# sanhue903/CUDA_Selection_Criteria

Measured on AMD Instinct MI355X. Metric: sketch pair-comparisons/sec (N genomes x m buckets), higher is better.
Workload: dtype u64; 1 GPU; cfg3: 10000 genomes, smh_a m=512, tau=0.8; mode smh_a; bands 64 x 8 rows; pair space sharded by query rows over 1 GPU(s), selected pairs all_gathered; n_genomes=10000, m=512, algo=sig, criterion=smh_a, selected_pairs=45000, stage1_survivors=45000, n_ranks_seen=1, stage2_grouping=label order

## Files before the change

cuda_selection_criteria_amd/csrc/abi_context.inc:

```

extern "C" {

const char* selhip_version(void) { return "selhip 0.1 (gfx950)"; }

int selhip_device_count(void) {
    int cnt = 0;
    if (hipGetDeviceCount(&cnt) != hipSuccess) return 0;
    return cnt;
}

const char* selhip_last_error(const selhip_ctx* ctx) {
    if (ctx) return ctx->err.c_str();
    return g_last_error.c_str();
}

int selhip_ctx_create(selhip_ctx** out, int device) {
    if (!out) return SELHIP_E_BADARG;
    *out = nullptr;
    int rc = check_device(nullptr);
    if (rc) return rc;
    int cnt = 0;
    (void)hipGetDeviceCount(&cnt);
    if (device < 0 || device >= cnt) { set_err(nullptr, "device %d out of range (0..%d)", device, cnt - 1); return SELHIP_E_BADARG; }
    HIPCHK(nullptr, hipSetDevice(device));
    hipDeviceProp_t prop;
    HIPCHK(nullptr, hipGetDeviceProperties(&prop, device));
    if (std::strncmp(prop.gcnArchName, "gfx950", 6) != 0) {
        set_err(nullptr, "device %d is %s; this library is built for gfx950 only", device, prop.gcnArchName);
        return SELHIP_E_NODEVICE;
    }
    selhip_ctx* c = new selhip_ctx();
    c->device = device;
    c->dev_cus = prop.multiProcessorCount;
    *out = c;
    return SELHIP_OK;
}

void selhip_ctx_destroy(selhip_ctx* c) {
    if (!c) return;
    (void)hipSetDevice(c->device);
    (void)hipStreamSynchronize(c->stream);
    drain_timers(c);
    c->own_hll.release(); c->own_aux.release(); c->own_cards.release();
    c->ecard.release(); c->hi.release(); c->pc.release(); c->seg_cnt.release(); c->surv.release();
    c->counts.release(); c->results.release(); c->self_pairs.release();
    c->aux_il.release(); c->cand.release(); c->sigQ.release(); c->sigT.release(); c->sigP.release(); c->sigG.release(); c->fin.release(); c->own_aux_hll.release();
    c->hj_keys_in.release(); c->hj_keys_out.release(); c->hj_vals_in.release(); c->hj_vals_out.release(); c->hj_tmp.release();
    c->csr_cnt.release(); c->csr_start.release(); c->grouped.release(); c->scan_tmp.release();
    c->hll_bs.release(); c->hll_bs_max.release(); c->hll_gmax.release(); c->small_bar.release();
    release_queries(c);
    if (c->h_pc) (void)hipHostFree(c->h_pc);
    if (c->st_stage1) {
        (void)hipStreamDestroy(c->st_stage1);
        (void)hipEventDestroy(c->ev_start); (void)hipEventDestroy(c->ev_end);
    }
    delete c;
}

int selhip_ctx_set_stream(selhip_ctx* c, void* hip_stream) {
    if (!c) return SELHIP_E_BADARG;
    if (c->stream != (hipStream_t)hip_stream && c->pc.p) {
        (void)hipStreamSynchronize(c->stream);
        c->pc_dirty = true;
    }
    c->stream = (hipStream_t)hip_stream;
    return SELHIP_OK;
}

int selhip_ctx_set_fp_mode(selhip_ctx* c, int fp_mode) {
    if (!c || (fp_mode != SELHIP_FP_FMA && fp_mode != SELHIP_FP_STRICT)) return SELHIP_E_BADARG;
    c->fp_mode = fp_mode;
    return SELHIP_OK;
}

int selhip_ctx_set_row_interleave(selhip_ctx* c, int block_rows, int n_parts, int part) {
    if (!c) return SELHIP_E_BADARG;
    if (n_parts <= 1) { c->il_parts = 1; c->il_part = 0; return SELHIP_OK; }
    if (block_rows < 32 || block_rows % 32 || part < 0 || part >= n_parts) {
        set_err(&c->err, "row interleave: block_rows must be a multiple of 32 (>= 32) and 0 <= part < n_parts");
        return SELHIP_E_BADARG;
    }
    c->il_block = block_rows; c->il_parts = n_parts; c->il_part = part;
// ... 60 lines not shown
        return SELHIP_OK;
    }
    if (!std::strcmp(name, "group_label")) {
        if (value < -1 || value > 1) { set_err(&c->err, "group_label must be -1 (automatic), 0 or 1"); return SELHIP_E_BADARG; }
        c->group_label = value;
        return SELHIP_OK;
    }
    if (!std::strcmp(name, "hist_run")) {
        if (value < 0 || value > 1024) { set_err(&c->err, "hist_run must be in [0, 1024] (0 = automatic)"); return SELHIP_E_BADARG; }
        c->hist_run = value;
        return SELHIP_OK;
    }
    if (!std::strcmp(name, "hist_pad")) {
        if (value < 0 || value > 48 * 1024) { set_err(&c->err, "hist_pad must be in [0, 49152]"); return SELHIP_E_BADARG; }
        c->hist_pad = value;
        return SELHIP_OK;
    }
    if (!std::strcmp(name, "query_join_tile")) {
        if (value != 16 && value != 32) { set_err(&c->err, "query_join_tile must be 16 or 32"); return SELHIP_E_BADARG; }
        c->query_join_tile = value;
        return SELHIP_OK;
    }
    if (!std::strcmp(name, "timed_kernel")) {
        if (value < 0 || value > 1) { set_err(&c->err, "timed_kernel must be 0 (stage-1 kernel) or 1 (stage 2a)"); return SELHIP_E_BADARG; }
        c->timed_kernel = value;
        return SELHIP_OK;
    }
    if (!std::strcmp(name, "hist_algo")) {
        if (value < -1 || value > 1) { set_err(&c->err, "hist_algo must be -1 (automatic), 0 (byte rows, LDS histogram) or 1 (bit planes)"); return SELHIP_E_BADARG; }
        c->hist_algo = value;
        if (value == 0) c->hll_khi = 0;
        return SELHIP_OK;
    }
    if (!std::strcmp(name, "hist_dense_degree")) {
        if (value < -1 || value > (1 << 20)) { set_err(&c->err, "hist_dense_degree must be in [-1, 2^20] (-1 = never)"); return SELHIP_E_BADARG; }
        c->hist_dense_degree = value;
        return SELHIP_OK;
    }
    if (!std::strcmp(name, "hist_bs_blocks")) {
        if (value < 8 || value > 65536 || value % 8) { set_err(&c->err, "hist_bs_blocks must be a multiple of 8 in [8, 65536]"); return SELHIP_E_BADARG; }
        c->hist_bs_blocks = value;
        return SELHIP_OK;
    }
    if (!std::strcmp(name, "hist_blocks")) {
        if (value < 8 || value > 65536 || value % 8) { set_err(&c->err, "hist_blocks must be a multiple of 8 in [8, 65536]"); return SELHIP_E_BADARG; }
        c->hist_blocks = value;
        return SELHIP_OK;
    }
    set_err(&c->err, "unknown parameter '%s'", name);
    return SELHIP_E_BADARG;
}

int selhip_ctx_get_param(const selhip_ctx* c, const char* name, int* value) {
    if (!c || !name || !value) return SELHIP_E_BADARG;
    if (!std::strcmp(name, "hll_khi"))          { *value = c->hll_khi; return SELHIP_OK; }
    if (!std::strcmp(name, "hist_bitplanes"))   { *value = use_bitslices(c) ? 1 : 0; return SELHIP_OK; }
    if (!std::strcmp(name, "label_order"))      { *value = label_order(c) ? 1 : 0; return SELHIP_OK; }
    if (!std::strcmp(name, "join_tile_rows"))   { *value = join_tile_rows(c); return SELHIP_OK; }
    if (!std::strcmp(name, "join_form_used"))   { *value = c->join_form_used; return SELHIP_OK; }
    if (!std::strcmp(name, "chunks"))           { *value = c->n_chunks_last; return SELHIP_OK; }
    if (!std::strcmp(name, "small_pass_used"))  { *value = c->small_used ? 1 : 0; return SELHIP_OK; }
    if (!std::strcmp(name, "query_db_sig_builds")) { *value = c->q.db_sig_builds; return SELHIP_OK; }
    return SELHIP_E_BADARG;
}

int selhip_ctx_set_candidate_begin(selhip_ctx* c, int64_t k_min) {
    if (!c) return SELHIP_E_BADARG;
    if (k_min < 0 || k_min > c->n) { set_err(&c->err, "candidate_begin %lld outside [0, n]", (long long)k_min); return SELHIP_E_BADARG; }
    c->cand_begin = k_min;
    return SELHIP_OK;
}

int selhip_ctx_set_stage2_grouping(selhip_ctx* c, int enable) {
    if (!c) return SELHIP_E_BADARG;
    c->group_stage2 = enable != 0;
    return SELHIP_OK;
}

int selhip_ctx_set_pipeline(selhip_ctx* c, int chunks) {
    if (!c || chunks < -1 || chunks > kMaxChunks) return SELHIP_E_BADARG;
    c->pipeline = chunks;
    return SELHIP_OK;
}

int selhip_ctx_set_criterion(selhip_ctx* c, int criterion) {
    if (!c || criterion < SELHIP_CRIT_SMH_A || criterion > SELHIP_CRIT_HLL_A_SMH_A) return SELHIP_E_BADARG;
    c->criterion = criterion;
    return SELHIP_OK;
}

int selhip_ctx_upload_aux_hll(selhip_ctx* c, const uint8_t* h_aux_hll, int p_aux) {
    if (!c || !h_aux_hll || p_aux < 4 || p_aux > kMaxAuxP) return SELHIP_E_BADARG;
    if (!c->d_hll && c->n) { set_err(&c->err, "upload the primary sketches first"); return SELHIP_E_STATE; }
    HIPCHK(&c->err, hipSetDevice(c->device));
    const size_t bytes = (size_t)c->n << p_aux;
    HIPCHK(&c->err, c->own_aux_hll.ensure(bytes ? bytes : 1));
    if (bytes) HIPCHK(&c->err, hipMemcpyAsync(c->own_aux_hll.p, h_aux_hll, bytes, hipMemcpyHostToDevice, c->stream));
    HIPCHK(&c->err, hipStreamSynchronize(c->stream));
    c->d_aux_hll = c->own_aux_hll.p; c->p_aux = p_aux;
    return SELHIP_OK;
}

int selhip_ctx_attach_aux_hll(selhip_ctx* c, const uint8_t* d_aux_hll, int p_aux) {
    if (!c || !d_aux_hll || p_aux < 4 || p_aux > kMaxAuxP) return SELHIP_E_BADARG;
    c->d_aux_hll = d_aux_hll; c->p_aux = p_aux;
    return SELHIP_OK;
}

static int validate_shape(selhip_ctx* c, int64_t n, int m, int p) {
    if (n < 0 || n > 0x7FFFFFF0ll) { set_err(&c->err, "n_genomes %lld out of range", (long long)n); return SELHIP_E_BADARG; }
    if (m <= 0) { set_err(&c->err, "m must be > 0"); return SELHIP_E_BADARG; }
    if (p < 4 || p > 20) { set_err(&c->err, "p_hll %d out of range [4,20]", p); return SELHIP_E_BADARG; }
    return SELHIP_OK;
}

static int after_sketches(selhip_ctx* c, const double* cards_src, bool cards_on_host) {
    c->hll_khi = 0;
    if (c->n == 0) return SELHIP_OK;
    if (c->p == 14 && c->hist_algo != 0) {
        HIPCHK(&c->err, c->hll_bs.ensure((size_t)c->n * kBsGenomeDwords));
        HIPCHK(&c->err, c->hll_bs_max.ensure(1));
        HIPCHK(&c->err, c->hll_gmax.ensure((size_t)c->n));
        const int rc = build_bitslices(&c->err, c->stream, c->d_hll, c->n, c->hll_bs.p, c->hll_gmax.p, c->hll_bs_max.p, &c->hll_khi);
        if (rc) return rc;
    }
    if (!cards_src) {
        HIPCHK(&c->err, c->own_cards.ensure((size_t)c->n));
        int rc = compute_cards(c, c->d_hll, c->n, c->p, c->own_cards.p);
        if (rc) return rc;
        c->d_cards = c->own_cards.p;
    } else if (cards_on_host) {
        for (int64_t i = 0; i < c->n; ++i) {
            double v = cards_src[i];
            if (!(v >= 0.0) || !(v < 9.2e18)) { set_err(&c->err, "cards[%lld] = %g is not a finite value in [0, 2^63)", (long long)i, v); return SELHIP_E_BADARG; }
            if (i && v < cards_src[i - 1]) { set_err(&c->err, "cards are not in ascending order at rank %lld", (long long)i); return SELHIP_E_BADARG; }
        }
        HIPCHK(&c->err, c->own_cards.ensure((size_t)c->n));
        HIPCHK(&c->err, hipMemcpyAsync(c->own_cards.p, cards_src, (size_t)c->n * sizeof(double), hipMemcpyHostToDevice, c->stream));
        c->d_cards = c->own_cards.p;
    } else {
        c->d_cards = cards_src;
    }
    HIPCHK(&c->err, hipStreamSynchronize(c->stream));
    return SELHIP_OK;
}

int selhip_ctx_upload(selhip_ctx* c, const uint8_t* h_hll, const uint64_t* h_aux, const double* h_cards,
                      int64_t n, int m, int p_hll) {
    if (!c) return SELHIP_E_BADARG;
    HIPCHK(&c->err, hipSetDevice(c->device));
    int rc = validate_shape(c, n, m, p_hll);
    if (rc) return rc;
    if (n > 0 && (!h_hll || !h_aux)) { set_err(&c->err, "null sketch pointer"); return SELHIP_E_BADARG; }
    c->n = n; c->m = m; c->p = p_hll; c->have_run = false; c->pending = false; c->cand_begin = 0; c->sig_key = 0; c->small_pass_failed = false;
    const size_t hb = (size_t)1 << p_hll;
    if (n > 0) {
// ... 242 lines not shown
```

cuda_selection_criteria_amd/csrc/host_context.hpp:

```cpp
#pragma once

namespace {

thread_local std::string g_last_error = "";

void set_err(std::string* dst, const char* fmt, ...) {
    char buf[512];
    va_list ap;
    va_start(ap, fmt);
    vsnprintf(buf, sizeof buf, fmt, ap);
    va_end(ap);
    if (dst) *dst = buf;
    g_last_error = buf;
}

#define HIPCHK(ctx_err, expr)                                                                  \
    do {                                                                                       \
        hipError_t e__ = (expr);                                                               \
        if (e__ != hipSuccess) {                                                               \
            set_err(ctx_err, "%s failed: %s (%s:%d)", #expr, hipGetErrorString(e__), __FILE__, __LINE__); \
            return SELHIP_E_HIP;                                                               \
        }                                                                                      \
    } while (0)

// ... 59 lines not shown
    DevBuf<selhip_int2_t> surv;
    DevBuf<uint32_t> counts;
    DevBuf<selhip_pair_t> results;
    DevBuf<selhip_int2_t> self_pairs;
    DevBuf<selhip_int2_t> cand;
    DevBuf<selhip_int2_t> fin;
    const uint8_t* d_aux_hll = nullptr;
    DevBuf<uint8_t> own_aux_hll;
    int p_aux = 0;
    int criterion = 0;
    DevBuf<u64> aux_il;
    DevBuf<uint32_t> sigQ, sigT, sigP, sigG;
    DevBuf<u64> hj_keys_in, hj_keys_out;
    DevBuf<int> hj_vals_in, hj_vals_out;
    DevBuf<char> hj_tmp;
    DevBuf<int> csr_cnt, csr_start;
    DevBuf<selhip_int2_t> grouped;
    DevBuf<char> scan_tmp;
    size_t scan_tmp_stride = 0;
    PassCounters* h_pc = nullptr;
    hipStream_t st_stage1 = nullptr;
    hipEvent_t ev_start = nullptr, ev_end = nullptr;
    int n_chunks_last = 1;
    int pipeline = -1;
    int64_t cand_begin = 0;
    int il_block = 128, il_parts = 1, il_part = 0;
    int hist_pad = 0;
    int hist_run = 0, hist_blocks = kHistSpanBlocks;
    DevBuf<uint32_t> hll_bs;
    DevBuf<u64> small_bar;
    DevBuf<uint8_t> hll_gmax;
    DevBuf<int> hll_bs_max;
    int hll_khi = 0;
    int hist_algo = -1;
    int hist_dense_degree = 32;
    int hist_bs_blocks = 2048;
    int group_label = -1;
    int verify_fb = 0;
    int join_wpb = 4;
    int join_db = 1;
    int join_tri = 0;
    int join_form = 2;
    int join_form_used = -1;
    int join_t = 0;
    int join_bits = 16;
    int join_q = 1;
    long long enum_pairs = kEnumPairs;
    int sig_tile_g = 16;
    int sig_cache = 0;
    long long sig_key = 0;
    int sig_tile = 1;
    int init_cap = 0;
    int join_qt = 0;
    bool group_stage2 = true;
    int small_pass = -1;
    bool small_used = false, small_pass_failed = false;
    int group_min_n = 2048;

    bool have_run = false, pending = false;
    int mode = 0, algo = 0, n_rows = 0, n_bands = 0;
    float tau_f = 0;
    int64_t row_begin = 0, row_end = 0;
    PassCounters last{};

    struct QuerySet {
        int64_t n = -1;
// ... 125 lines not shown
```

cuda_selection_criteria_amd/csrc/host_pass.hpp:

```cpp
#pragma once

namespace {

template <int NCH, int LOG2R>
hipError_t launch_stream(selhip_ctx* c, const StageIO& io, const RowMap& rm) {
    constexpr int Q = kQueryVgprBudget / NCH;
    const int n = (int)c->n;
    const long long n_tiles_ll = rm.n_tiles(Q);
    if (n_tiles_ll > 0x7FFFFFFFll) return hipErrorInvalidValue;
    const int n_tiles = (int)n_tiles_ll;
    const int chunk_base = ((rm.row_begin + 1) / kChunk) * kChunk;
    const int n_chunks = (n - chunk_base + kChunk - 1) / kChunk;
    if (n_tiles <= 0 || n_chunks <= 0) return hipSuccess;
    const long long blocks = (long long)n_tiles * n_chunks;
    if (blocks > 0x7FFFFFFFll) return hipErrorInvalidValue;
    hipLaunchKernelGGL((smh_stream_kernel<NCH, LOG2R>), dim3((unsigned)blocks), dim3(kBlock), 0, io.st,
                       reinterpret_cast<const u64x2*>(c->aux_il.p), n, c->hi.p, c->pcb,
                       rm, n_tiles, chunk_base, io.surv, io.cap, io.pc);
    return hipGetLastError();
}

template <int NCH, int LOG2R>
hipError_t launch_stream_r(selhip_ctx* c, const StageIO& io, int l, const RowMap& rm) {
    if (l == LOG2R) return launch_stream<NCH, LOG2R>(c, io, rm);
// ... 233 lines not shown
    size_t tmp_bytes = c->hj_tmp.cap;
    const unsigned end_bit = 32u + (unsigned)ilog2(n_bands) + 1u;
    e = rocprim::radix_sort_pairs(c->hj_tmp.p, tmp_bytes, c->hj_keys_in.p, c->hj_keys_out.p, c->hj_vals_in.p, c->hj_vals_out.p,
                                  (size_t)total, 0u, end_bit, io.st);
    if (e != hipSuccess) return e;
    hipLaunchKernelGGL(run_emit_kernel, dim3(grid_for((u64)total, kBlock, 8192)), dim3(kBlock), 0, io.st,
                       c->hj_keys_out.p, c->hj_vals_out.p, total, c->sigQ.p, n_bands, c->d_aux, c->m, n_rows, n_bands,
                       n, c->hi.p, c->pcb, rm, io.surv, io.cap, io.pc);
    return hipGetLastError();
}

template <int MODE>
hipError_t launch_select(bool fma, hipStream_t st, unsigned grid, const uint32_t* counts, const u64* n_dev, u64 n_host,
                         u64 cap, int p, double* est, const selhip_int2_t* pairs, const u64* ecard, double tau,
                         selhip_pair_t* results, u64 results_cap, PassCounters* pc,
                         selhip_result_t* rf32, int* out_count, u64 chunk_off = 0, u64 chunk_len = ~0ull) {
    const double rs = relerr_scaled_for(p);
    if (fma)
        hipLaunchKernelGGL((ertl_select_kernel<true, MODE>), dim3((grid + kWavesPerBlock - 1) / kWavesPerBlock), dim3(kBlock), 0, st, counts, n_dev, n_host, cap,
                           p, rs, est, pairs, ecard, tau, results, results_cap, pc, rf32, out_count, chunk_off, chunk_len);
    else
        hipLaunchKernelGGL((ertl_select_kernel<false, MODE>), dim3((grid + kWavesPerBlock - 1) / kWavesPerBlock), dim3(kBlock), 0, st, counts, n_dev, n_host, cap,
                           p, rs, est, pairs, ecard, tau, results, results_cap, pc, rf32, out_count, chunk_off, chunk_len);
    return hipGetLastError();
}

unsigned grid_for(u64 items, unsigned per_block, unsigned max_blocks) {
    u64 b = (items + per_block - 1) / per_block;
    if (b < 1) b = 1;
    if (b > max_blocks) b = max_blocks;
    return (unsigned)b;
}

hipError_t launch_hist_bs(int khi, unsigned blocks, hipStream_t st, const uint32_t* bs, const uint8_t* gmax, const selhip_int2_t* list, const u64* count,
                          u64 cap, uint32_t* counts, u64 off, u64 window, int run, u64 dense_pairs) {
#define SELHIP_BS_LAUNCH(NB) hipLaunchKernelGGL((hll_union_hist_bs_kernel<NB>), dim3(blocks), dim3(kBlock), 0, st, bs, gmax, list, count, cap, counts, off, window, run, dense_pairs)
    if (khi <= 16)      SELHIP_BS_LAUNCH(4);
    else if (khi <= 32) SELHIP_BS_LAUNCH(5);
    else                SELHIP_BS_LAUNCH(6);
#undef SELHIP_BS_LAUNCH
    return hipGetLastError();
}

int build_bitslices(std::string* err, hipStream_t st, const uint8_t* d_hll, int64_t n, uint32_t* d_bs, uint8_t* d_gmax, int* d_max, int* khi) {
    HIPCHK(err, hipMemsetAsync(d_max, 0, sizeof(int), st));
    hipLaunchKernelGGL(hll_bitslice_kernel, dim3(grid_for((u64)n, kWavesPerBlock, 8192)), dim3(kBlock), 0, st, d_hll, (long long)n, d_bs, d_gmax, d_max);
    HIPCHK(err, hipGetLastError());
    int mx = 0;
    HIPCHK(err, hipMemcpyAsync(&mx, d_max, sizeof(int), hipMemcpyDeviceToHost, st));
    HIPCHK(err, hipStreamSynchronize(st));
    *khi = mx + 1;
    return SELHIP_OK;
}

bool use_bitslices(const selhip_ctx* c) { return c->p == 14 && c->hll_khi > 0 && c->hist_algo != 0; }

int compute_cards(selhip_ctx* c, const uint8_t* d_hll, int64_t n, int p, double* d_out) {
    if (n <= 0) return SELHIP_OK;
    HIPCHK(&c->err, c->self_pairs.ensure((size_t)n));
    HIPCHK(&c->err, c->counts.ensure((size_t)n * 64));
    hipLaunchKernelGGL(iota_pairs_kernel, dim3((unsigned)((n + 255) / 256)), dim3(256), 0, c->stream, c->self_pairs.p, (int)n);
    HIPCHK(&c->err, hipGetLastError());
    hipLaunchKernelGGL(hll_union_hist_kernel, dim3(grid_for((u64)n, kWavesPerBlock, 4096)), dim3(kBlock), 0, c->stream,
                       d_hll, p, c->self_pairs.p, (const u64*)nullptr, (u64)n, (u64)n, c->counts.p);
    HIPCHK(&c->err, hipGetLastError());
    HIPCHK(&c->err, launch_select<0>(c->fp_mode == SELHIP_FP_FMA, c->stream, grid_for((u64)n, kWave, 8192), c->counts.p,
                                     nullptr, (u64)n, (u64)n, p, d_out, nullptr, nullptr, 0.0, nullptr, 0, nullptr,
                                     nullptr, nullptr));
    return SELHIP_OK;
}

float sigma_p_of(int p) {
    switch (p) {
        case 4: return (float)(1.106 / std::sqrt((double)(1 << p)));
        case 5: return (float)(1.07 / std::sqrt((double)(1 << p)));
        case 6: return (float)(1.054 / std::sqrt((double)(1 << p)));
        case 7: return (float)(1.046 / std::sqrt((double)(1 << p)));
    }
    return (float)(1.039 / std::sqrt((double)(1 << p)));
}

long long pair_bound(long long n, long long rb, long long re) {
    long long cnt = 0;
    const long long rows = re - rb;
    cnt = rows * (n - 1) - (rb + re - 1) * rows / 2;
    return cnt < 0 ? 0 : cnt;
}

// ... 98 lines not shown
            HIPCHK(&c->err, hipGetLastError());
        } else if (label) {
            const unsigned row_blocks = (unsigned)((n + kBlock - 1) / kBlock);
            hipLaunchKernelGGL(csr_label_sum_kernel, dim3(row_blocks), dim3(kBlock), 0, st, cnt, lab, n, gsum);
            HIPCHK(&c->err, hipGetLastError());
            size_t tmp_bytes = c->scan_tmp_stride;
            HIPCHK(&c->err, rocprim::exclusive_scan(ch.scan_tmp, tmp_bytes, gsum, ch.csr_start, 0, (size_t)n, rocprim::plus<int>(), st));
            hipLaunchKernelGGL(csr_label_assign_kernel, dim3(row_blocks), dim3(kBlock), 0, st, cnt, lab, n, ch.csr_start, gsum);
            HIPCHK(&c->err, hipGetLastError());
            hipLaunchKernelGGL(csr_fill_kernel, dim3(512), dim3(kBlock), 0, st, final_list, final_count, final_cap, gsum, fill, ch.grouped);
            HIPCHK(&c->err, hipGetLastError());
        } else if (n <= kSmallScanMax) {
            if ((size_t)n * sizeof(int) > 48 * 1024)
                HIPCHK(&c->err, hipFuncSetAttribute((const void*)csr_scan_fill_kernel, hipFuncAttributeMaxDynamicSharedMemorySize, kSmallScanMax * 4));
            hipLaunchKernelGGL(csr_scan_fill_kernel, dim3(256), dim3(1024), (size_t)n * sizeof(int), st, cnt, n,
                               final_list, final_count, final_cap, fill, ch.grouped);
            HIPCHK(&c->err, hipGetLastError());
        } else {
            size_t tmp_bytes = c->scan_tmp_stride;
            HIPCHK(&c->err, rocprim::exclusive_scan(ch.scan_tmp, tmp_bytes, cnt, ch.csr_start, 0, (size_t)n, rocprim::plus<int>(), st));
            hipLaunchKernelGGL(csr_fill_kernel, dim3(512), dim3(kBlock), 0, st, final_list, final_count, final_cap,
                               ch.csr_start, fill, ch.grouped);
            HIPCHK(&c->err, hipGetLastError());
        }
        final_list = ch.grouped;
    }
    for (u64 off = 0; off < final_cap; off += ch.window) {
        {
            TimerScope t(c, T_HIST, st);
            if (use_bitslices(c))
                HIPCHK(&c->err, launch_hist_bs(c->hll_khi, (unsigned)c->hist_bs_blocks, st, c->hll_bs.p, c->hll_gmax.p, final_list, final_count, final_cap, ch.counts, off, ch.window,
                                               c->hist_run > 0 ? c->hist_run : (grouped ? 4 : 1),
                                               grouped && c->hist_dense_degree >= 0
                                                   ? (u64)c->hist_dense_degree * (u64)std::max<long long>(1, ((long long)ch.re - ch.rb) / std::max(1, c->il_parts)) : ~0ull));
            else if (c->p == 14)
                hipLaunchKernelGGL(hll_union_hist_runs_kernel, dim3(c->hist_blocks), dim3(kWave), (size_t)c->hist_pad, st,
                                   c->d_hll, final_list, final_count, final_cap, ch.counts, off, ch.window,
                                   c->hist_run > 0 ? c->hist_run : (grouped && label_order(c) ? 4 : 1));
            else
                hipLaunchKernelGGL(hll_union_hist_kernel, dim3(2048), dim3(kBlock), 0, st,
                                   c->d_hll, c->p, final_list, final_count, (u64)0, final_cap, ch.counts, off, ch.window);
            HIPCHK(&c->err, hipGetLastError());
        }
        TimerScope t(c, T_SELECT, st);
        HIPCHK(&c->err, launch_select<1>(c->fp_mode == SELHIP_FP_FMA, st, 4096, ch.counts, final_count, 0,
                                         final_cap, c->p, nullptr, final_list, c->ecard.p, tau,
                                         c->results.p, (u64)c->results.cap, pc0, nullptr, nullptr, off, ch.window));
    }
    return SELHIP_OK;
}

int enqueue_chain(selhip_ctx* c, const Chain& ch, int rb, int re, double tau, bool use_hash, bool use_sig, bool count_in_verify,
                  PassCounters* pc0) {
    const StageIO& io = ch.io;
    RowMap rm = row_map(c, rb, re);
    if (c->il_parts <= 1) rm = row_map(c, ch.rb, ch.re);
    else { rm.row_begin = ch.rb; rm.row_end = ch.re; }
    {
        TimerScope t(c, T_STAGE1, io.st);
        if (use_hash)     HIPCHK(&c->err, launch_stage1_hashjoin(c, io, c->n_rows, c->n_bands, rm));
        else if (use_sig) HIPCHK(&c->err, launch_stage1_sig(c, io, c->n_rows, c->n_bands, rm));
        else              HIPCHK(&c->err, launch_stage1(c, io, c->n_rows, c->n_bands, rm));
    }
    const selhip_int2_t* final_list = io.surv;
    const u64* final_count = &io.pc->n_survivors;
    u64 final_cap = io.cap;
    if (c->criterion == SELHIP_CRIT_HLL_A_SMH_A) {
// ... 273 lines not shown
```

cuda_selection_criteria_amd/csrc/kernel_hllbs.cuh:

```cuda
#pragma once

namespace {

constexpr int kBsPlanes = 6;
constexpr int kBsPlaneDwords = 512;
constexpr int kBsGenomeDwords = kBsPlanes * kBsPlaneDwords;

__global__ __launch_bounds__(kBlock)
void hll_bitslice_kernel(const uint8_t* __restrict__ hll, long long n, uint32_t* __restrict__ bs, uint8_t* __restrict__ gmax,
                         int* __restrict__ max_val) {
    const int lane = threadIdx.x & (kWave - 1);
    uint32_t mx_all = 0;
    for (long long g = (long long)blockIdx.x * kWavesPerBlock + threadIdx.x / kWave; g < n; g += (long long)gridDim.x * kWavesPerBlock) {
        const uint32_t* row = reinterpret_cast<const uint32_t*>(hll + g * 16384);
        uint32_t* dst = bs + g * kBsGenomeDwords;
        uint32_t mx = 0;
#pragma unroll 1
        for (int o = 0; o < 8; ++o) {
            uint32_t d[8];
#pragma unroll
            for (int jj = 0; jj < 8; ++jj) d[jj] = row[(o * 8 + jj) * kWave + lane] & 0x3F3F3F3Fu;
            uint32_t out[kBsPlanes];
#pragma unroll
            for (int b = 0; b < kBsPlanes; ++b) out[b] = 0;
#pragma unroll
            for (int jj = 0; jj < 8; ++jj) {
                const uint32_t w = d[jj];
                mx = max(max(mx, w & 0xFFu), max((w >> 8) & 0xFFu, max((w >> 16) & 0xFFu, w >> 24)));
#pragma unroll
                for (int b = 0; b < kBsPlanes; ++b) out[b] |= ((w >> b) & 0x01010101u) << jj;
            }
#pragma unroll
            for (int b = 0; b < kBsPlanes; ++b) dst[b * kBsPlaneDwords + o * kWave + lane] = out[b];
        }
#pragma unroll
        for (int s = 32; s > 0; s >>= 1) mx = max(mx, (uint32_t)__shfl_xor((int)mx, s, kWave));
        if (lane == 0) gmax[g] = (uint8_t)mx;
        mx_all = max(mx_all, mx);
    }
    if (lane == 0 && mx_all) atomicMax(max_val, (int)mx_all);
}

template <int NB>
__device__ __forceinline__ void bs_load(const uint32_t* __restrict__ bs, int g, int lane, uint32_t (&r)[NB][8]) {
    const uint4* p = reinterpret_cast<const uint4*>(bs + (size_t)g * kBsGenomeDwords);
#pragma unroll
    for (int b = 0; b < NB; ++b) {
        const uint4 lo = p[b * (kBsPlaneDwords / 4) + lane], hi = p[b * (kBsPlaneDwords / 4) + kWave + lane];
        r[b][0] = lo.x; r[b][1] = lo.y; r[b][2] = lo.z; r[b][3] = lo.w;
        r[b][4] = hi.x; r[b][5] = hi.y; r[b][6] = hi.z; r[b][7] = hi.w;
    }
}

template <int TBL>
__device__ __forceinline__ uint32_t bs_op3(uint32_t a, uint32_t b, uint32_t c) { return __builtin_amdgcn_bitop3_b32(a, b, c, TBL); }
__device__ __forceinline__ void bs_count(uint32_t& acc, uint32_t mask) {
    asm("v_bcnt_u32_b32 %0, %1, %0" : "+v"(acc) : "v"(mask));
}

template <int NB, int G>
__device__ __forceinline__ uint32_t bs_group_node(const uint32_t (&M)[NB], const uint32_t (&pre)[4]) {
    constexpr int s1 = (G & 2) ? 0xCC : 0x33, s0 = (G & 1) ? 0xAA : 0x55;
    if constexpr (NB == 4)      return bs_op3<((G & 2) ? 0xF0 : 0x0F) & ((G & 1) ? 0xCC : 0x33)>(M[3], M[2], M[2]);
    else if constexpr (NB == 5) return bs_op3<((G & 4) ? 0xF0 : 0x0F) & s1 & s0>(M[4], M[3], M[2]);
    else                        return bs_op3<0xF0 & s1 & s0>(pre[G >> 2], M[3], M[2]);
}

template <int NB, int G0, int G, int GEND>
__device__ __forceinline__ void bs_groups(const uint32_t (&M)[NB], const uint32_t (&pre)[4], uint32_t (&A)[GEND - G0], uint32_t (&B)[GEND - G0],
                                          uint32_t (&C0)[GEND - G0], uint32_t (&C1)[GEND - G0]) {
    if constexpr (G < GEND) {
        const uint32_t node = bs_group_node<NB, G>(M, pre);
        bs_count(A[G - G0], node);
        bs_count(B[G - G0], node & M[1]);
        bs_count(C0[G - G0], bs_op3<0xF0 & 0x33 & 0xAA>(node, M[1], M[0]));
// ... 9 lines not shown
    uint32_t A[NG], B[NG], C0[NG], C1[NG];
#pragma unroll
    for (int v = 0; v < NG; ++v) { A[v] = 0; B[v] = 0; C0[v] = 0; C1[v] = 0; }
#pragma unroll
    for (int c = 0; c < 8; ++c) {
        uint32_t g = 0;
#pragma unroll
        for (int b = 0; b < NB; ++b) g = bs_op3<0xB2>(xa[b][c], yb[b][c], g);
        uint32_t M[NB];
#pragma unroll
        for (int b = 0; b < NB; ++b) M[b] = bs_op3<0xCA>(g, xa[b][c], yb[b][c]);
        uint32_t pre[4] = {0u, 0u, 0u, 0u};
        if constexpr (NB == 6) {
            if constexpr (G0 < 4 && GE > 0)   pre[0] = bs_op3<0x0F & 0x33>(M[5], M[4], M[4]);
            if constexpr (G0 < 8 && GE > 4)   pre[1] = bs_op3<0x0F & 0xCC>(M[5], M[4], M[4]);
            if constexpr (G0 < 12 && GE > 8)  pre[2] = bs_op3<0xF0 & 0x33>(M[5], M[4], M[4]);
            if constexpr (G0 < 16 && GE > 12) pre[3] = bs_op3<0xF0 & 0xCC>(M[5], M[4], M[4]);
        }
        bs_groups<NB, G0, G0, GE>(M, pre, A, B, C0, C1);
    }
#pragma unroll
    for (int v = 0; v < NG; ++v) {
        P[2 * (G0 + v)]     = (A[v] - B[v] - C0[v]) | (C0[v] << 16);
        P[2 * (G0 + v) + 1] = (B[v] - C1[v]) | (C1[v] << 16);
    }
}

template <int CTRL>
__device__ __forceinline__ uint32_t bs_dpp(uint32_t v) {
    return (uint32_t)__builtin_amdgcn_update_dpp(0, (int)v, CTRL, 0xF, 0xF, true);
}
constexpr int kDppRowMirror = 0x140, kDppRowHalfMirror = 0x141, kDppQuad3210 = 0x1B, kDppQuad1032 = 0xB1;

__device__ __forceinline__ uint32_t bs_reduce16(const uint32_t (&P)[16], int lane) {
    uint32_t Q[8], R[4];
#pragma unroll
    for (int j = 0; j < 8; ++j) {
        const auto s = __builtin_amdgcn_permlane32_swap(P[2 * j], P[2 * j + 1], false, false);
        Q[j] = s[0] + s[1];
    }
#pragma unroll
    for (int j = 0; j < 4; ++j) {
        const auto s = __builtin_amdgcn_permlane16_swap(Q[2 * j], Q[2 * j + 1], false, false);
        R[j] = s[0] + s[1];
    }
    const bool h = (lane & 8) != 0, q = (lane & 4) != 0;
    const uint32_t t0 = R[0] + bs_dpp<kDppRowMirror>(R[0]), t1 = R[1] + bs_dpp<kDppRowMirror>(R[1]);
    const uint32_t t2 = R[2] + bs_dpp<kDppRowMirror>(R[2]), t3 = R[3] + bs_dpp<kDppRowMirror>(R[3]);
    const uint32_t S0 = h ? t1 : t0, S1 = h ? t3 : t2;
    const uint32_t u0 = S0 + bs_dpp<kDppRowHalfMirror>(S0), u1 = S1 + bs_dpp<kDppRowHalfMirror>(S1);
    const uint32_t U = q ? u1 : u0;
    const uint32_t V = U + bs_dpp<kDppQuad3210>(U);
    return V + bs_dpp<kDppQuad1032>(V);
}
__device__ __forceinline__ int bs_pidx(int lane) {
    const int r = lane >> 4;
    return 4 * (2 * ((lane >> 2) & 1) + ((lane >> 3) & 1)) + (((r & 1) << 1) | (r >> 1));
}

template <int NB>
__device__ __forceinline__ uint32_t bs_pair_hist(const uint32_t (&xa)[NB][8], const uint32_t (&yb)[NB][8], int kp, int lane) {
    constexpr int NP = NB == 6 ? 32 : 16;
    uint32_t P[NP];
#pragma unroll
    for (int v = 0; v < NP; ++v) P[v] = 0u;
    if constexpr (NB == 4) {
        bs_decode<NB, 0, 4, NP>(xa, yb, P);
    } else {
        bs_decode<NB, 0, 6, NP>(xa, yb, P);
        if (kp > 24) bs_decode<NB, 6, 8, NP>(xa, yb, P);
        if constexpr (NB == 6) {
            if (kp > 32) bs_decode<NB, 8, 12, NP>(xa, yb, P);
            if (kp > 48) bs_decode<NB, 12, 16, NP>(xa, yb, P);
        }
    }
    uint32_t lo[16];
#pragma unroll
    for (int v = 0; v < 16; ++v) lo[v] = P[v];
    uint32_t tot = bs_reduce16(lo, lane);
    if constexpr (NP > 16) {
        uint32_t tot_hi = 0;
        if (kp > 32) {
#pragma unroll
            for (int v = 0; v < 16; ++v) lo[v] = P[16 + v];
            tot_hi = bs_reduce16(lo, lane);
        }
        tot = (lane & 2) ? tot_hi : tot;
    } else {
        tot = (lane & 2) ? 0u : tot;
    }
    return tot;
}

template <int NB>
__global__ __launch_bounds__(kBlock, NB <= 5 ? 4 : 2)
void hll_union_hist_bs_kernel(const uint32_t* __restrict__ bs, const uint8_t* __restrict__ gmax, const selhip_int2_t* __restrict__ pairs,
                              const u64* __restrict__ n_pairs_dev, u64 cap, uint32_t* __restrict__ counts,
                              u64 chunk_off, u64 chunk_len, int run_len, u64 dense_pairs) {
    const int lane = threadIdx.x & (kWave - 1);
    const int wave = threadIdx.x / kWave;
    u64 n_pairs = *n_pairs_dev;
    if (n_pairs > cap) n_pairs = cap;
    n_pairs = n_pairs > chunk_off ? min(n_pairs - chunk_off, chunk_len) : 0;
    pairs += chunk_off;
    u64 blocks_active = gridDim.x;
    {
        const u64 resident = 1024ull * (NB <= 5 ? 4 : 2);
        if (n_pairs <= 8 * resident) {
            const u64 waves = min(resident, max(n_pairs, (u64)64));
            blocks_active = min((u64)gridDim.x, ((waves + 8 * kWavesPerBlock - 1) / (8 * kWavesPerBlock)) * 8);
        }
    }
    if (blockIdx.x >= blocks_active) return;
    const u64 stride = (blocks_active >> 3) * kWavesPerBlock;
    const int my_bin = ((lane & 2) ? 32 : 0) + 2 * bs_pidx(lane) + (lane & 1);
    const bool dense = n_pairs >= dense_pairs;
    const uint32_t xcd = blockIdx.x & 7u;
    const u64 waves_active = 8 * stride;
    const bool short_list = blocks_active < gridDim.x;
    const u64 per_wave = short_list ? (n_pairs + waves_active - 1) / waves_active : n_pairs / (16 * stride);
    run_len = dense ? kWave : (int)max((u64)1, min((u64)min(run_len, short_list ? 2 : kWave), per_wave));
    const u64 n_tasks = (n_pairs + run_len - 1) / run_len;
    const u64 tasks_per_xcd = dense ? n_tasks : (n_tasks + 7) >> 3;
    const u64 t_begin = dense ? 0 : (u64)xcd * tasks_per_xcd, t_end = min(t_begin + tasks_per_xcd, n_tasks);
    int cur_x = -1;
    uint32_t xa[NB][8];
    for (u64 task = t_begin + (u64)(blockIdx.x >> 3) * kWavesPerBlock + wave; task < t_end; task += stride) {
        const u64 j0 = task * run_len;
        const int cnt = (int)min((u64)run_len, n_pairs - j0);
        selhip_int2_t pr{0, 0};
        if (lane < cnt) pr = pairs[j0 + lane];
        u64 mine = __ballot(lane < cnt && (!dense || (((uint32_t)pr.y * 0x9E3779B1u) >> 29) == xcd));
        while (mine) {
            const int src = (int)__builtin_ctzll(mine);
            mine &= mine - 1;
            const int px = __builtin_amdgcn_readlane(pr.x, src), py = __builtin_amdgcn_readlane(pr.y, src);
            uint32_t yb[NB][8];
            bs_load<NB>(bs, py, lane, yb);
            if (px != cur_x) { bs_load<NB>(bs, px, lane, xa); cur_x = px; }
            const int kp = max((int)gmax[px], (int)gmax[py]) + 1;
            const uint32_t tot = bs_pair_hist<NB>(xa, yb, kp, lane);
            counts[(j0 + src) * 64 + my_bin] = (lane & 1) ? (tot >> 16) : (tot & 0xFFFFu);
        }
    }
}


}
```

Measured before the change: 251.7 billion pairs/s.

## Handle high HLL register values via per-genome sparse lists in bit-plane histogram

Adds a preprocessing pass that finds a threshold t such that every genome has at most 128 registers with value >= t, then builds per-genome sparse lists of those registers. The union-histogram kernel is templated on t/4 groups: it decodes only the low value groups from the bit planes and merges the sparse high-value entries per pair through wave-local LDS bitmaps and bins. This aims to cut the bit-plane decode and reduction work for rare high values. In exchange it adds LDS use per wave, atomics, extra global reads for the lists, a host sync during setup, and more kernel instantiations.

```diff
diff --git a/cuda_selection_criteria_amd/csrc/abi_context.inc b/cuda_selection_criteria_amd/csrc/abi_context.inc
--- a/cuda_selection_criteria_amd/csrc/abi_context.inc
+++ b/cuda_selection_criteria_amd/csrc/abi_context.inc
@@ -48,6 +48,7 @@
     c->hj_keys_in.release(); c->hj_keys_out.release(); c->hj_vals_in.release(); c->hj_vals_out.release(); c->hj_tmp.release();
     c->csr_cnt.release(); c->csr_start.release(); c->grouped.release(); c->scan_tmp.release();
     c->hll_bs.release(); c->hll_bs_max.release(); c->hll_gmax.release(); c->small_bar.release();
+    c->hll_sparse.release(); c->hll_sparse_dev_t.release();
     release_queries(c);
     if (c->h_pc) (void)hipHostFree(c->h_pc);
     if (c->st_stage1) {
@@ -174,6 +175,11 @@
         if (value == 0) c->hll_khi = 0;
         return SELHIP_OK;
     }
+    if (!std::strcmp(name, "hist_sparse")) {
+        if (value < -1 || value > 1) { set_err(&c->err, "hist_sparse must be -1 (automatic), 0 (every value from the bit planes) or 1 (values >= the set's threshold from its sparse lists)"); return SELHIP_E_BADARG; }
+        c->hist_sparse = value;
+        return SELHIP_OK;
+    }
     if (!std::strcmp(name, "hist_dense_degree")) {
         if (value < -1 || value > (1 << 20)) { set_err(&c->err, "hist_dense_degree must be in [-1, 2^20] (-1 = never)"); return SELHIP_E_BADARG; }
         c->hist_dense_degree = value;
@@ -197,6 +203,7 @@
     if (!c || !name || !value) return SELHIP_E_BADARG;
     if (!std::strcmp(name, "hll_khi"))          { *value = c->hll_khi; return SELHIP_OK; }
     if (!std::strcmp(name, "hist_bitplanes"))   { *value = use_bitslices(c) ? 1 : 0; return SELHIP_OK; }
+    if (!std::strcmp(name, "hist_sparse_t"))    { *value = sparse_t_used(c); return SELHIP_OK; }
     if (!std::strcmp(name, "label_order"))      { *value = label_order(c) ? 1 : 0; return SELHIP_OK; }
     if (!std::strcmp(name, "join_tile_rows"))   { *value = join_tile_rows(c); return SELHIP_OK; }
     if (!std::strcmp(name, "join_form_used"))   { *value = c->join_form_used; return SELHIP_OK; }
@@ -257,13 +264,17 @@
 }
 
 static int after_sketches(selhip_ctx* c, const double* cards_src, bool cards_on_host) {
-    c->hll_khi = 0;
+    c->hll_khi = 0; c->hll_sparse_t = 0;
     if (c->n == 0) return SELHIP_OK;
     if (c->p == 14 && c->hist_algo != 0) {
         HIPCHK(&c->err, c->hll_bs.ensure((size_t)c->n * kBsGenomeDwords));
         HIPCHK(&c->err, c->hll_bs_max.ensure(1));
         HIPCHK(&c->err, c->hll_gmax.ensure((size_t)c->n));
-        const int rc = build_bitslices(&c->err, c->stream, c->d_hll, c->n, c->hll_bs.p, c->hll_gmax.p, c->hll_bs_max.p, &c->hll_khi);
+        int rc = build_bitslices(&c->err, c->stream, c->d_hll, c->n, c->hll_bs.p, c->hll_gmax.p, c->hll_bs_max.p, &c->hll_khi);
+        if (rc) return rc;
+        HIPCHK(&c->err, c->hll_sparse.ensure((size_t)c->n * kBsSparseCap));
+        HIPCHK(&c->err, c->hll_sparse_dev_t.ensure(1));
+        rc = build_sparse_lists(&c->err, c->stream, c->hll_bs.p, c->n, c->hll_sparse.p, c->hll_sparse_dev_t.p, &c->hll_sparse_t);
         if (rc) return rc;
     }
     if (!cards_src) {
diff --git a/cuda_selection_criteria_amd/csrc/host_context.hpp b/cuda_selection_criteria_amd/csrc/host_context.hpp
--- a/cuda_selection_criteria_amd/csrc/host_context.hpp
+++ b/cuda_selection_criteria_amd/csrc/host_context.hpp
@@ -115,6 +115,10 @@
     DevBuf<uint8_t> hll_gmax;
     DevBuf<int> hll_bs_max;
     int hll_khi = 0;
+    DevBuf<uint32_t> hll_sparse;
+    DevBuf<int> hll_sparse_dev_t;
+    int hll_sparse_t = 0;
+    int hist_sparse = -1;
     int hist_algo = -1;
     int hist_dense_degree = 32;
     int hist_bs_blocks = 2048;
diff --git a/cuda_selection_criteria_amd/csrc/host_pass.hpp b/cuda_selection_criteria_amd/csrc/host_pass.hpp
--- a/cuda_selection_criteria_amd/csrc/host_pass.hpp
+++ b/cuda_selection_criteria_amd/csrc/host_pass.hpp
@@ -289,14 +289,52 @@
     return (unsigned)b;
 }
 
+template <int NB>
+void launch_hist_bs_nb(int g1, unsigned blocks, hipStream_t st, const uint32_t* bs, const uint8_t* gmax, const uint32_t* lists, const selhip_int2_t* list,
+                       const u64* count, u64 cap, uint32_t* counts, u64 off, u64 window, int run, u64 dense_pairs) {
+#define SELHIP_BS_LAUNCH(G1) hipLaunchKernelGGL((hll_union_hist_bs_kernel<NB, G1>), dim3(blocks), dim3(kBlock), 0, st, bs, gmax, lists, list, count, cap, \
+                                                counts, off, window, run, dense_pairs)
+    switch (g1) {
+        case 1: SELHIP_BS_LAUNCH(1); return;
+        case 2: SELHIP_BS_LAUNCH(2); return;
+        case 3: SELHIP_BS_LAUNCH(3); return;
+    }
+    if constexpr (NB > 4) {
+        switch (g1) {
+            case 4: SELHIP_BS_LAUNCH(4); return;
+            case 5: SELHIP_BS_LAUNCH(5); return;
+        }
+    }
+    if constexpr (NB > 5) {
+        if (g1 == 6) { SELHIP_BS_LAUNCH(6); return; }
+    }
+    SELHIP_BS_LAUNCH(0);
+#undef SELHIP_BS_LAUNCH
+}
 hipError_t launch_hist_bs(int khi, unsigned blocks, hipStream_t st, const uint32_t* bs, const uint8_t* gmax, const selhip_int2_t* list, const u64* count,
-                          u64 cap, uint32_t* counts, u64 off, u64 window, int run, u64 dense_pairs) {
-#define SELHIP_BS_LAUNCH(NB) hipLaunchKernelGGL((hll_union_hist_bs_kernel<NB>), dim3(blocks), dim3(kBlock), 0, st, bs, gmax, list, count, cap, counts, off, window, run, dense_pairs)
-    if (khi <= 16)      SELHIP_BS_LAUNCH(4);
-    else if (khi <= 32) SELHIP_BS_LAUNCH(5);
-    else                SELHIP_BS_LAUNCH(6);
-#undef SELHIP_BS_LAUNCH
-    return hipGetLastError();
+                          u64 cap, uint32_t* counts, u64 off, u64 window, int run, u64 dense_pairs, int sparse_t = 0, const uint32_t* lists = nullptr) {
+    const int g1 = sparse_t > 0 && sparse_t < khi && lists ? sparse_t / 4 : 0;
+    if (khi <= 16)      launch_hist_bs_nb<4>(g1, blocks, st, bs, gmax, lists, list, count, cap, counts, off, window, run, dense_pairs);
+    else if (khi <= 32) launch_hist_bs_nb<5>(g1, blocks, st, bs, gmax, lists, list, count, cap, counts, off, window, run, dense_pairs);
+    else                launch_hist_bs_nb<6>(g1, blocks, st, bs, gmax, lists, list, count, cap, counts, off, window, run, dense_pairs);
+    return hipGetLastError();
+}
+
+int build_sparse_lists(std::string* err, hipStream_t st, const uint32_t* d_bs, int64_t n, uint32_t* d_lists, int* d_t, int* t) {
+    *t = 0;
+    if (n <= 0) return SELHIP_OK;
+    HIPCHK(err, hipMemsetAsync(d_t, 0, sizeof(int), st));
+    hipLaunchKernelGGL(hll_sparse_t_kernel, dim3(grid_for((u64)n, kWavesPerBlock, 8192)), dim3(kBlock), 0, st, d_bs, (long long)n, d_t);
+    HIPCHK(err, hipGetLastError());
+    int need = 0;
+    HIPCHK(err, hipMemcpyAsync(&need, d_t, sizeof(int), hipMemcpyDeviceToHost, st));
+    HIPCHK(err, hipStreamSynchronize(st));
+    if (need < 4 || need > kBsSparseMaxT) return SELHIP_OK;
+    hipLaunchKernelGGL(hll_sparse_list_kernel, dim3(grid_for((u64)n, kWavesPerBlock, 8192)), dim3(kBlock), 0, st, d_bs, (long long)n, need, d_lists);
+    HIPCHK(err, hipGetLastError());
+    HIPCHK(err, hipStreamSynchronize(st));
+    *t = need;
+    return SELHIP_OK;
 }
 
 int build_bitslices(std::string* err, hipStream_t st, const uint8_t* d_hll, int64_t n, uint32_t* d_bs, uint8_t* d_gmax, int* d_max, int* khi) {
@@ -311,6 +349,13 @@
 }
 
 bool use_bitslices(const selhip_ctx* c) { return c->p == 14 && c->hll_khi > 0 && c->hist_algo != 0; }
+constexpr size_t kSparseMaxPlaneBytes = (size_t)192 << 20;
+int sparse_t_used(const selhip_ctx* c) {
+    if (!use_bitslices(c) || !c->hist_sparse || c->hll_sparse_t >= c->hll_khi) return 0;
+    if (c->hist_sparse < 0 && (size_t)c->n * kBsGenomeDwords * sizeof(uint32_t) > kSparseMaxPlaneBytes) return 0;
+    if (c->hll_sparse_t > 20 && c->hll_khi <= 32) return 0;
+    return c->hll_sparse_t;
+}
 
 int compute_cards(selhip_ctx* c, const uint8_t* d_hll, int64_t n, int p, double* d_out) {
     if (n <= 0) return SELHIP_OK;
@@ -475,7 +520,8 @@
                 HIPCHK(&c->err, launch_hist_bs(c->hll_khi, (unsigned)c->hist_bs_blocks, st, c->hll_bs.p, c->hll_gmax.p, final_list, final_count, final_cap, ch.counts, off, ch.window,
                                                c->hist_run > 0 ? c->hist_run : (grouped ? 4 : 1),
                                                grouped && c->hist_dense_degree >= 0
-                                                   ? (u64)c->hist_dense_degree * (u64)std::max<long long>(1, ((long long)ch.re - ch.rb) / std::max(1, c->il_parts)) : ~0ull));
+                                                   ? (u64)c->hist_dense_degree * (u64)std::max<long long>(1, ((long long)ch.re - ch.rb) / std::max(1, c->il_parts)) : ~0ull,
+                                               sparse_t_used(c), c->hll_sparse.p));
             else if (c->p == 14)
                 hipLaunchKernelGGL(hll_union_hist_runs_kernel, dim3(c->hist_blocks), dim3(kWave), (size_t)c->hist_pad, st,
                                    c->d_hll, final_list, final_count, final_cap, ch.counts, off, ch.window,
diff --git a/cuda_selection_criteria_amd/csrc/kernel_hllbs.cuh b/cuda_selection_criteria_amd/csrc/kernel_hllbs.cuh
--- a/cuda_selection_criteria_amd/csrc/kernel_hllbs.cuh
+++ b/cuda_selection_criteria_amd/csrc/kernel_hllbs.cuh
@@ -41,6 +41,83 @@
     if (lane == 0 && mx_all) atomicMax(max_val, (int)mx_all);
 }
 
+constexpr int kBsSparseCap = 128;
+constexpr int kBsSparseMaxT = 24;
+constexpr uint32_t kBsSparseNone = 0xFFFFFFFFu;
+
+__device__ __forceinline__ uint32_t bs_ge4k(const uint32_t (&p)[kBsPlanes], int k) {
+    uint32_t borrow = 0;
+#pragma unroll
+    for (int i = 0; i < 4; ++i) borrow = ((k >> i) & 1) ? (~p[2 + i] | borrow) : (~p[2 + i] & borrow);
+    return ~borrow;
+}
+
+__global__ __launch_bounds__(kBlock)
+void hll_sparse_t_kernel(const uint32_t* __restrict__ bs, long long n, int* __restrict__ t_need) {
+    const int lane = threadIdx.x & (kWave - 1);
+    int t_all = 0;
+    for (long long g = (long long)blockIdx.x * kWavesPerBlock + threadIdx.x / kWave; g < n; g += (long long)gridDim.x * kWavesPerBlock) {
+        const uint32_t* src = bs + g * kBsGenomeDwords;
+        int cnt[6] = {0, 0, 0, 0, 0, 0};
+#pragma unroll 1
+        for (int o = 0; o < kBsPlaneDwords / kWave; ++o) {
+            uint32_t p[kBsPlanes];
+#pragma unroll
+            for (int b = 0; b < kBsPlanes; ++b) p[b] = src[b * kBsPlaneDwords + o * kWave + lane];
+#pragma unroll
+            for (int k = 1; k <= 6; ++k) cnt[k - 1] += __popc(bs_ge4k(p, k));
+        }
+        int t = kBsSparseMaxT + 4;
+#pragma unroll
+        for (int k = 6; k >= 1; --k) {
+            int s = cnt[k - 1];
+#pragma unroll
+            for (int d = 32; d > 0; d >>= 1) s += __shfl_xor(s, d, kWave);
+            if (s <= kBsSparseCap) t = 4 * k;
+        }
+        t_all = max(t_all, t);
+    }
+    if (lane == 0 && t_all) atomicMax(t_need, t_all);
+}
+
+__global__ __launch_bounds__(kBlock)
+void hll_sparse_list_kernel(const uint32_t* __restrict__ bs, long long n, int t, uint32_t* __restrict__ lists) {
+    const int lane = threadIdx.x & (kWave - 1);
+    for (long long g = (long long)blockIdx.x * kWavesPerBlock + threadIdx.x / kWave; g < n; g += (long long)gridDim.x * kWavesPerBlock) {
+        const uint32_t* src = bs + g * kBsGenomeDwords;
+        uint32_t* dst = lists + g * kBsSparseCap;
+        int base = 0;
+#pragma unroll 1
+        for (int o = 0; o < kBsPlaneDwords / kWave; ++o) {
+            const int d = o * kWave + lane;
+            uint32_t p[kBsPlanes];
+#pragma unroll
+            for (int b = 0; b < kBsPlanes; ++b) p[b] = src[b * kBsPlaneDwords + d];
+            uint32_t h = bs_ge4k(p, t >> 2);
+            const int cnt = __popc(h);
+            int incl = cnt;
+#pragma unroll
+            for (int s = 1; s < kWave; s <<= 1) {
+                const int v = __shfl_up(incl, s, kWave);
+                if (lane >= s) incl += v;
+            }
+            int off = base + incl - cnt;
+            while (h) {
+                const int j = __builtin_ctz(h);
+                h &= h - 1;
+                uint32_t v = 0;
+#pragma unroll
+                for (int b = 0; b < kBsPlanes; ++b) v |= ((p[b] >> j) & 1u) << b;
+                if (off < kBsSparseCap) dst[off] = ((uint32_t)(d * 32 + j) << 8) | v;
+                ++off;
+            }
+            base += __shfl(incl, kWave - 1, kWave);
+        }
+        for (int i = lane; i < kBsSparseCap; i += kWave)
+            if (i >= base) dst[i] = kBsSparseNone;
+    }
+}
+
 template <int NB>
 __device__ __forceinline__ void bs_load(const uint32_t* __restrict__ bs, int g, int lane, uint32_t (&r)[NB][8]) {
     const uint4* p = reinterpret_cast<const uint4*>(bs + (size_t)g * kBsGenomeDwords);
@@ -116,23 +193,29 @@
 }
 constexpr int kDppRowMirror = 0x140, kDppRowHalfMirror = 0x141, kDppQuad3210 = 0x1B, kDppQuad1032 = 0xB1;
 
+template <int NV = 16>
 __device__ __forceinline__ uint32_t bs_reduce16(const uint32_t (&P)[16], int lane) {
     uint32_t Q[8], R[4];
 #pragma unroll
     for (int j = 0; j < 8; ++j) {
+        if (2 * j >= NV) { Q[j] = 0u; continue; }
         const auto s = __builtin_amdgcn_permlane32_swap(P[2 * j], P[2 * j + 1], false, false);
         Q[j] = s[0] + s[1];
     }
 #pragma unroll
     for (int j = 0; j < 4; ++j) {
+        if (4 * j >= NV) { R[j] = 0u; continue; }
         const auto s = __builtin_amdgcn_permlane16_swap(Q[2 * j], Q[2 * j + 1], false, false);
         R[j] = s[0] + s[1];
     }
     const bool h = (lane & 8) != 0, q = (lane & 4) != 0;
-    const uint32_t t0 = R[0] + bs_dpp<kDppRowMirror>(R[0]), t1 = R[1] + bs_dpp<kDppRowMirror>(R[1]);
-    const uint32_t t2 = R[2] + bs_dpp<kDppRowMirror>(R[2]), t3 = R[3] + bs_dpp<kDppRowMirror>(R[3]);
+    const uint32_t t0 = R[0] + bs_dpp<kDppRowMirror>(R[0]);
+    const uint32_t t1 = NV > 4 ? R[1] + bs_dpp<kDppRowMirror>(R[1]) : 0u;
+    const uint32_t t2 = NV > 8 ? R[2] + bs_dpp<kDppRowMirror>(R[2]) : 0u;
+    const uint32_t t3 = NV > 12 ? R[3] + bs_dpp<kDppRowMirror>(R[3]) : 0u;
     const uint32_t S0 = h ? t1 : t0, S1 = h ? t3 : t2;
-    const uint32_t u0 = S0 + bs_dpp<kDppRowHalfMirror>(S0), u1 = S1 + bs_dpp<kDppRowHalfMirror>(S1);
+    const uint32_t u0 = S0 + bs_dpp<kDppRowHalfMirror>(S0);
+    const uint32_t u1 = NV > 8 ? S1 + bs_dpp<kDppRowHalfMirror>(S1) : 0u;
     const uint32_t U = q ? u1 : u0;
     const uint32_t V = U + bs_dpp<kDppQuad3210>(U);
     return V + bs_dpp<kDppQuad1032>(V);
@@ -176,10 +259,68 @@
     return tot;
 }
 
-template <int NB>
+struct alignas(16) BsSparseLds {
+    uint32_t bits[kBsPlaneDwords];
+    uint32_t bins[64];
+    uint8_t first[kBsPlaneDwords];
+    uint8_t val[kBsSparseCap];
+};
+
+__device__ __forceinline__ uint32_t bs_sparse_row(BsSparseLds* sp, const uint32_t* __restrict__ lists, int x, int lane, int my_bin) {
+    const uint32_t e0 = lists[(size_t)x * kBsSparseCap + lane], e1 = lists[(size_t)x * kBsSparseCap + kWave + lane];
+    uint4* bits4 = reinterpret_cast<uint4*>(sp->bits);
+    bits4[2 * lane] = make_uint4(0u, 0u, 0u, 0u);
+    bits4[2 * lane + 1] = make_uint4(0u, 0u, 0u, 0u);
+    __builtin_amdgcn_fence(__ATOMIC_RELEASE, "wavefront");
+    __builtin_amdgcn_wave_barrier();
+    __builtin_amdgcn_fence(__ATOMIC_ACQUIRE, "wavefront");
+#pragma unroll
+    for (int h = 0; h < 2; ++h) {
+        const uint32_t e = h ? e1 : e0;
+        if (e != kBsSparseNone) {
+            const uint32_t r = e >> 8;
+            atomicOr(&sp->bits[r >> 5], 1u << (r & 31));
+            atomicAdd(&sp->bins[e & 63], 1u);
+            sp->val[h * kWave + lane] = (uint8_t)(e & 63);
+        }
+    }
+    __builtin_amdgcn_fence(__ATOMIC_RELEASE, "wavefront");
+    __builtin_amdgcn_wave_barrier();
+    __builtin_amdgcn_fence(__ATOMIC_ACQUIRE, "wavefront");
+#pragma unroll
+    for (int h = 0; h < 2; ++h) {
+        const uint32_t e = h ? e1 : e0;
+        if (e != kBsSparseNone) {
+            const uint32_t r = e >> 8;
+            sp->first[r >> 5] = (uint8_t)(h * kWave + lane - __popc(sp->bits[r >> 5] & ((1u << (r & 31)) - 1u)));
+        }
+    }
+    const uint32_t hA = sp->bins[my_bin];
+    sp->bins[my_bin] = 0u;
+    __builtin_amdgcn_fence(__ATOMIC_RELEASE, "wavefront");
+    __builtin_amdgcn_wave_barrier();
+    __builtin_amdgcn_fence(__ATOMIC_ACQUIRE, "wavefront");
+    return hA;
+}
+
+__device__ __forceinline__ void bs_sparse_entry(BsSparseLds* sp, uint32_t e) {
+    if (e == kBsSparseNone) return;
+    const uint32_t r = e >> 8, v = e & 63, w = sp->bits[r >> 5], below = w & ((1u << (r & 31)) - 1u);
+    if ((w >> (r & 31)) & 1u) {
+        const uint32_t av = sp->val[sp->first[r >> 5] + __popc(below)];
+        if (v > av) {
+            atomicAdd(&sp->bins[v], 1u);
+            atomicSub(&sp->bins[av], 1u);
+        }
+    } else {
+        atomicAdd(&sp->bins[v], 1u);
+    }
+}
+
+template <int NB, int G1>
 __global__ __launch_bounds__(kBlock, NB <= 5 ? 4 : 2)
-void hll_union_hist_bs_kernel(const uint32_t* __restrict__ bs, const uint8_t* __restrict__ gmax, const selhip_int2_t* __restrict__ pairs,
-                              const u64* __restrict__ n_pairs_dev, u64 cap, uint32_t* __restrict__ counts,
+void hll_union_hist_bs_kernel(const uint32_t* __restrict__ bs, const uint8_t* __restrict__ gmax, const uint32_t* __restrict__ lists,
+                              const selhip_int2_t* __restrict__ pairs, const u64* __restrict__ n_pairs_dev, u64 cap, uint32_t* __restrict__ counts,
                               u64 chunk_off, u64 chunk_len, int run_len, u64 dense_pairs) {
     const int lane = threadIdx.x & (kWave - 1);
     const int wave = threadIdx.x / kWave;
@@ -209,6 +350,13 @@
     const u64 t_begin = dense ? 0 : (u64)xcd * tasks_per_xcd, t_end = min(t_begin + tasks_per_xcd, n_tasks);
     int cur_x = -1;
     uint32_t xa[NB][8];
+    BsSparseLds* sp = nullptr;
+    uint32_t hA = 0;
+    if constexpr (G1 > 0) {
+        __shared__ BsSparseLds sp_block[kWavesPerBlock];
+        sp = &sp_block[wave];
+        sp->bins[my_bin] = 0u;
+    }
     for (u64 task = t_begin + (u64)(blockIdx.x >> 3) * kWavesPerBlock + wave; task < t_end; task += stride) {
         const u64 j0 = task * run_len;
         const int cnt = (int)min((u64)run_len, n_pairs - j0);
@@ -221,13 +369,32 @@
             const int px = __builtin_amdgcn_readlane(pr.x, src), py = __builtin_amdgcn_readlane(pr.y, src);
             uint32_t yb[NB][8];
             bs_load<NB>(bs, py, lane, yb);
-            if (px != cur_x) { bs_load<NB>(bs, px, lane, xa); cur_x = px; }
-            const int kp = max((int)gmax[px], (int)gmax[py]) + 1;
-            const uint32_t tot = bs_pair_hist<NB>(xa, yb, kp, lane);
-            counts[(j0 + src) * 64 + my_bin] = (lane & 1) ? (tot >> 16) : (tot & 0xFFFFu);
-        }
-    }
-}
-
-
-}
+            if constexpr (G1 == 0) {
+                if (px != cur_x) { bs_load<NB>(bs, px, lane, xa); cur_x = px; }
+                const int kp = max((int)gmax[px], (int)gmax[py]) + 1;
+                const uint32_t tot = bs_pair_hist<NB>(xa, yb, kp, lane);
+                counts[(j0 + src) * 64 + my_bin] = (lane & 1) ? (tot >> 16) : (tot & 0xFFFFu);
+            } else {
+                const uint32_t eb0 = lists[(size_t)py * kBsSparseCap + lane], eb1 = lists[(size_t)py * kBsSparseCap + kWave + lane];
+                if (px != cur_x) { bs_load<NB>(bs, px, lane, xa); hA = bs_sparse_row(sp, lists, px, lane, my_bin); cur_x = px; }
+                uint32_t P[16];
+#pragma unroll
+                for (int v = 0; v < 16; ++v) P[v] = 0u;
+                bs_decode<NB, 0, G1, 16>(xa, yb, P);
+                const uint32_t tot = bs_reduce16<2 * G1>(P, lane);
+                bs_sparse_entry(sp, eb0);
+                bs_sparse_entry(sp, eb1);
+                __builtin_amdgcn_fence(__ATOMIC_RELEASE, "wavefront");
+                __builtin_amdgcn_wave_barrier();
+                __builtin_amdgcn_fence(__ATOMIC_ACQUIRE, "wavefront");
+                const uint32_t s = sp->bins[my_bin];
+                sp->bins[my_bin] = 0u;
+                const uint32_t dense_cnt = (lane & 2) ? 0u : ((lane & 1) ? (tot >> 16) : (tot & 0xFFFFu));
+                counts[(j0 + src) * 64 + my_bin] = dense_cnt + hA + s;
+            }
+        }
+    }
+}
+
+
+}
```

After: 266.6 billion pairs/s (median of 6 runs). 1.06x the previous value.
